# khangklj/Video2Music

Hardware: AMD Instinct MI355X
Metric: chord_tokens_per_sec_generated (higher is better)
Workload: dtype f32; 1 GPU; AMT 6+6 layers d_model=512 H=8 dff=1024 rpr, seq=1024, batch=32 clips/GPU x 300-frame video features (F=1287), feedback-greedy (G2) generate incl. video encode; global_batch=32, seq_len=1024, parallelism=dp1

## Files before the change

### include/amt_hip.h

```cpp
#ifndef AMT_HIP_H
#define AMT_HIP_H
#include <stdint.h>

#define AMT_ABI_VERSION 14

#ifdef __cplusplus
extern "C" {
#endif

typedef struct amt_handle amt_handle;

typedef struct amt_config {
    int32_t n_layers;
    int32_t num_heads;
    int32_t d_model;
    int32_t dim_feedforward;
    int32_t max_sequence_video;
    int32_t max_sequence_chord;
    int32_t total_vf_dim;
    int32_t max_batch;
} amt_config;

const char* amt_last_error(void);
int32_t amt_abi_version(void);
// ... 75 lines not shown
typedef struct amt_decode_gemm_args {
    const float* x;  int32_t ldx;
    const float* x2; int32_t ldx2;
    int32_t K1, K;
    const float* w_low;  const float* bias_low;  const float* resid; int32_t relu;
    const float* w_high; const float* bias_high;
    int32_t n_low, n_high;
    int32_t pro;
    const float* fold_g; const float* fold_c; const float* ln_w; const float* ln_b;
    float* y_low; float* y_high;
    float* scratch_low; float* scratch_high;
    int32_t B; float eps;
} amt_decode_gemm_args;
int32_t amt_decode_gemm_ex_fwd(const amt_decode_gemm_args* a, void* stream);
int32_t amt_decode_gemm_ex_lean(const amt_decode_gemm_args* a);
int32_t amt_gqa_fwd(const float* query, const float* key, const float* value,
                    const float* wq, const float* bq, const float* wk, const float* bk, const float* wv, const float* bv,
                    const float* ln_w, const float* ln_b, const float* wo, const float* bo,
                    float* out, float* scratch, int32_t L, int32_t S, int32_t B, int32_t E, int32_t query_heads,
                    int32_t kv_heads, int32_t is_causal, float ln_eps, void* stream);
int32_t amt_gqa_rope_fwd(const float* query, const float* key, const float* value,
                         const float* wq, const float* bq, const float* wk, const float* bk, const float* wv, const float* bv,
                         const float* ln_w, const float* ln_b, const float* wo, const float* bo,
                         float* out, float* scratch, int32_t L, int32_t S, int32_t B, int32_t E, int32_t query_heads,
                         int32_t kv_heads, int32_t is_causal, float ln_eps, const float* rope_cache, int32_t cache_rows,
                         int32_t cache_half, void* stream);
int64_t amt_moe_scratch_floats(int32_t n_tok, int32_t d, int32_t dff, int32_t n_exp);
int32_t amt_moe_fwd(const float* x, const float* gate_w, const float* gate_b,
                    const float* w1, const float* b1, const float* wg, const float* bg, const float* w2, const float* b2,
                    const float* sw1, const float* sb1, const float* swg, const float* sbg, const float* sw2, const float* sb2,
// ... 191 lines not shown
```

### video2music_amd/_lib.py

```python
import ctypes as C
import os

_HERE = os.path.dirname(os.path.abspath(__file__))
LIB_PATH = os.environ.get("AMT_LIB") or os.path.join(_HERE, "lib", "libamt_hip.so")


class AmtError(RuntimeError):
    pass


class AmtConfig(C.Structure):
    _fields_ = [("n_layers", C.c_int32), ("num_heads", C.c_int32), ("d_model", C.c_int32),
                ("dim_feedforward", C.c_int32), ("max_sequence_video", C.c_int32),
                ("max_sequence_chord", C.c_int32), ("total_vf_dim", C.c_int32), ("max_batch", C.c_int32)]


_P = C.c_void_p
_I = C.c_int32
_F = C.c_float


class DecodeGemmArgs(C.Structure):
    _fields_ = [("x", _P), ("ldx", _I), ("x2", _P), ("ldx2", _I), ("K1", _I), ("K", _I),
                ("w_low", _P), ("bias_low", _P), ("resid", _P), ("relu", _I), ("w_high", _P), ("bias_high", _P),
# ... 41 lines not shown
    "amt_diff_subln_fwd": [_P, _P, _P, _P, _I, _I, _F, _F, _F, _P],
    "amt_add_fwd": [_P, _P, _P, C.c_int64, _P],
    "amt_row_scale_add_fwd": [_P, _P, _P, _P, _I, _I, _P],
    "amt_rope_fwd": [_P, _P, _P, _I, _I, _I, _I, _I, _P],
    "amt_rpr_attn_fwd": [_P, _P, _P, _P, _P, _I, _I, _I, _I, _I, _P],
    "amt_rpr_attn_nomask_fwd": [_P, _P, _P, _P, _P, _I, _I, _I, _I, _I, _P],
    "amt_cross_attn_fwd": [_P, _P, _P, _P, _I, _I, _I, _I, _I, _I, _P],
    "amt_attn_fwd": [_P, _P, _P, _P, C.POINTER(C.c_int64), _I, _I, _I, _I, _I, _I, _I, _F, _P],
    "amt_concat_features_fwd": [_P, _I, _P, _P, _I, _P, _I, _P, _I, _I, _P],
    "amt_chord_embed_fwd": [_P] * 9 + [_I, _I, _I, _P],
    "amt_attn_decode_fwd": [_P, _P, _P, _P, _P, _I, _I, _I, _I, _I, _I, _P],
    "amt_decode_linear_fwd": [_P, _P, _P, _P, _P, _P, _P, _P, _P, _I, _I, _I, _I, _F, _P],
    "amt_attn_decode_fold_fwd": [_P, _I] + [_P] * 10 + [_I, _I, _I, _I, _P, _I, _I, _I, _F, _F, _P],
    "amt_decode_gemm_ex_fwd": [C.POINTER(DecodeGemmArgs), _P],
    "amt_decode_gemm_ex_lean": [C.POINTER(DecodeGemmArgs)],
    "amt_gqa_fwd": [_P] * 15 + [_I] * 7 + [_F, _P],
    "amt_gqa_rope_fwd": [_P] * 15 + [_I] * 7 + [_F, _P, _I, _I, _P],
    "amt_moe_scratch_floats": [_I, _I, _I, _I],
    "amt_moe_fwd": [_P] * 19 + [_I] * 4 + [_P],
    "amt_moe_topk_scratch_floats": [_I, _I, _I, _I, _I],
    "amt_moe_topk_fwd": [_P] * 19 + [_I] * 5 + [_P],
    "amt_moe_train_scratch_floats": [_I, _I, _I, _I, _I, _I],
    "amt_moe_train_fwd": [_P] * 22 + [_I] * 6 + [_P],
    "amt_moe_bwd_ws_floats": [_I, _I, _I, _I, _I],
    "amt_moe_bwd": [_P] * 29 + [_I] * 8 + [_F, _P],
    "amt_moe_route_fwd": [_P, _P, _P, _P, _P, _I, _I, _I, _P],
    "amt_glu_expert_fwd": [_P] * 9 + [_I, _I, _I, _P],
    "amt_moe_combine_fwd": [_P, _P, _P, _P, _P, _F, _P, _I, _I, _P],
    "amt_moe_ep_dispatch_plan_fwd": [_P, _I, _I, _P, _P, _P, _P, _P],
    "amt_gather_rows_fwd": [_P, _P, _P, _I, _I, _P],
# ... 43 lines not shown
    "amt_diff_subln_bwd": [_P] * 10 + [_I, _I, _F, _F, _P],
    "amt_moe_train_fwd_balanced": [_P] * 22 + [_I] * 6 + [_P, _P, _F, _P],
    "amt_selective_scan_wide_ckpt_steps": [_I],
    "amt_selective_scan_wide_train_fwd": [_P, _I, _P, _I, _P, _P, _P, _P, _I, _P, _P, _I, _P, _I, _P, _I, _P, _I, _I, _I, _I, _I, _I, _P],
    "amt_selective_scan_wide_bwd_ws_floats": [_I, _I, _I, _I],
    "amt_selective_scan_wide_bwd": [_P, _I, _P, _I, _P, _I, _P, _P, _P, _P, _I, _P, _P, _I, _P, _I, _P, _P, _I, _P, _I, _P, _I, _P, _P, _I, _P, _P,
                                    _P, _I, _I, _I, _I, _I, _I, _P],
    "amt_silu_bwd": [_P, _P, _P, C.c_int64, _P],
}
_RESTYPES = {"amt_last_error": C.c_char_p, "amt_decode_step_bytes": C.c_int64, "amt_moe_scratch_floats": C.c_int64, "amt_moe_topk_scratch_floats": C.c_int64,
             "amt_v2_step_ws_floats": C.c_int64, "amt_v2_step_batch_ws_floats": C.c_int64, "amt_moe_ep_expert_scratch_floats": C.c_int64,
             "amt_chord_loss_ws_floats": C.c_int64, "amt_attn_bwd_ws_floats": C.c_int64, "amt_selective_scan_bwd_ws_floats": C.c_int64,
             "amt_dwconv1d_silu_bwd_ws_floats": C.c_int64, "amt_moe_train_scratch_floats": C.c_int64, "amt_moe_bwd_ws_floats": C.c_int64,
             "amt_glu_train_scratch_floats": C.c_int64, "amt_glu_bwd_ws_floats": C.c_int64,
             "amt_selective_scan_wide_bwd_ws_floats": C.c_int64}
_NO_STATUS = set(_RESTYPES) | {"amt_abi_version", "amt_v2_last_step_launches", "amt_gemm_route", "amt_attn_route", "amt_decode_gemm_ex_lean", "amt_moe_wgrad_splits",
                                  "amt_rmsnorm_bwd_blocks", "amt_diff_subln_bwd_blocks", "amt_selective_scan_wide_ckpt_steps"}

ABI_VERSION = 14

_lib = None


def load():
    global _lib
    if _lib is not None:
        return _lib
    import torch
    if not os.path.exists(LIB_PATH):
        raise AmtError(f"{LIB_PATH} is missing: the HIP extension is not built (run __graft_entry__.build()); "
                       "video2music_amd has no CPU fallback")
# ... 44 lines not shown
```

### video2music_amd/csrc/amt_api.hip

```cpp
#include <stdarg.h>
#include <stdio.h>
#include <stdlib.h>
#include <string.h>

#include <algorithm>
#include <map>
#include <string>
#include <vector>

#include "../../include/amt_hip.h"
#include "amt_common.h"
#include "kernels.h"

static thread_local char g_err[1024] = "";

void amt_set_error(const char* fmt, ...) {
    va_list ap;
    va_start(ap, fmt);
    vsnprintf(g_err, sizeof(g_err), fmt, ap);
    va_end(ap);
}

extern "C" const char* amt_last_error(void) { return g_err; }
extern "C" int32_t amt_abi_version(void) { return AMT_ABI_VERSION; }
// ... 54 lines not shown
    float* unif = nullptr;
    int use_unif = 0;
    int64_t *tokens = nullptr, *roots = nullptr, *attrs = nullptr;
    int genB = 0, genT = 0, genP = 0, beam = 0, mcN = 0, mcC = 2, steps_done = 0;
    int n_root = 15;
    bool chord_embed = false;
    bool causal_mask = true;
    const float* vis_resid = nullptr;
    int skip_mask = 0;
    bool fuse_head = true;
    bool short_attn = true;
    bool step_short = false;
    bool l0_tables = true;
    bool gemm_pipe = true;
    bool gemm_lean = true;
    bool scalar_stream = true;
    bool plain_chain = false;
    bool gen_active = false;
    struct GraphKey { int B, T, P, beam, mcN, mcC, S, nsteps, skip, pad, short_ctx, parity, gemm_pipe, spare, key_stream, gemm_front; float* logits; };
    struct GraphEntry { GraphKey key; hipGraphExec_t exec; hipGraph_t graph; };
    std::vector<GraphEntry> graphs;
    hipStream_t cap_stream = nullptr;
};

namespace {

template <typename T>
int32_t dev_alloc(amt_handle* h, T** out, size_t count) {
    void* p = nullptr;
    AMT_HIP(hipMalloc(&p, count * sizeof(T) + 256));
// ... 148 lines not shown
            a.fold_lnw = P.n3w; a.fold_lnb = P.n3b; a.xn = h->xa; a.new_kv = 1; a.k_new = Kc; a.v_new = Vc;
            a.eps = LN_EPS; a.q_scale = qscale;
        }
        if (l == 0 && fused_sp) {
            if ((rc = amt_launch_attn_decode_sample(a, *fused_sp, s))) return rc;
        } else if (!(h->skip_mask & 1)) {
            PROF_BEGIN();
            if ((rc = amt_launch_attn_decode(a, s))) return rc;
            PROF_END(0);
        }
        const float* r0 = l == 0 ? h->x_in : h->xa;
        DecodeGemmParams g1{};
        g1.B = B; g1.eps = LN_EPS; g1.scale = 1.f; g1.x = h->ob; g1.ldx = d; g1.x2 = r0; g1.ldx2 = d; g1.K1 = d; g1.K = 2 * d;
        g1.Wp = L.p_sao; g1.bias = L.sa_ob; g1.resid = r0; g1.ldr = d; g1.y = h->u1; g1.ldy = d;
        g1.n_split = d; g1.N = 2 * d; g1.Wp2 = L.pf_a; g1.bias2 = L.va + 2 * d; g1.y2 = h->qraw; g1.ldy2 = d;
        PROF_BEGIN();
        if ((rc = launch_step_gemm(h, g1, s))) return rc;
        PROF_END(2);
        AttnDecodeParams x{};
        x.k = Kx; x.v = Vx; x.o = h->ob; x.B = B; x.H = H; x.hd = hd; x.cap = h->kx_rows; x.n_keys = h->encS; x.lane_key_stream = h->scalar_stream ? 0 : 1;
        x.q = h->qraw; x.ldq = d; x.d = d; x.fold_u = h->u1; x.fold_g = L.va; x.fold_c = L.va + d;
        x.fold_lnw = L.n1w; x.fold_lnb = L.n1b; x.xn = h->xb; x.eps = LN_EPS; x.q_scale = qscale;
        if (!(h->skip_mask & 2)) {
            PROF_BEGIN();
            if ((rc = amt_launch_attn_decode(x, s))) return rc;
            PROF_END(1);
        }
        DecodeGemmParams g2{};
        g2.B = B; g2.eps = LN_EPS; g2.scale = 1.f; g2.x = h->ob; g2.ldx = d; g2.x2 = h->xb; g2.ldx2 = d; g2.K1 = d; g2.K = 2 * d;
        g2.Wp = L.p_cao; g2.bias = L.ca_ob; g2.resid = h->xb; g2.ldr = d; g2.y = h->u2; g2.ldy = d;
        g2.n_split = d; g2.N = d + dff; g2.Wp2 = L.pf_b; g2.bias2 = L.vb + 2 * dff; g2.y2 = h->hraw; g2.ldy2 = dff;
        PROF_BEGIN();
        if ((rc = launch_step_gemm(h, g2, s))) return rc;
        PROF_END(2);
        DecodeGemmParams g3{};
        g3.B = B; g3.eps = LN_EPS; g3.scale = 1.f; g3.pro = 1; g3.x = h->hraw; g3.ldx = dff; g3.x2 = h->u2; g3.ldx2 = d;
        g3.K1 = dff; g3.K = dff + d; g3.fold_g = L.vb; g3.fold_c = L.vb + dff; g3.ln_w = L.n2w; g3.ln_b = L.n2b;
// ... 79 lines not shown
                DecodeGemmParams c = f2;
                c.x = h->hb + k0; c.K = std::min(FFN_CHUNK, dff - k0); c.Wp = L.p_l2 + (size_t)cdiv(d, 16) * 16 * k0;
                if (k0) { c.bias = nullptr; c.resid = h->u3; }
                PROF_BEGIN();
                if ((rc = launch_step_gemm(h, c, s))) return rc;
                PROF_END(2);
            }
        }
    }
    return 0;
}

int32_t get_graph(amt_handle* h, int first_pos, int nsteps, float* logits_out, hipGraphExec_t* out) {
    const bool short_ctx = h->short_attn && first_pos + nsteps <= amt_attn_decode_stride(h->hd);
    amt_handle::GraphKey key{h->genB, h->genT, h->genP, h->beam, h->mcN, h->mcC, h->encS, nsteps, h->skip_mask | (h->fuse_head ? 4 : 0), h->use_unif,
                             short_ctx ? 1 : 0, first_pos & 1, h->gemm_pipe ? 1 : 0, h->l0_tables ? 1 : 0, h->scalar_stream ? 1 : 0, h->gemm_lean ? 1 : 0, logits_out};
    for (auto& g : h->graphs)
        if (memcmp(&g.key, &key, sizeof(key)) == 0) { *out = g.exec; return 0; }
    hipGraph_t graph;
    if (!h->cap_stream) AMT_HIP(hipStreamCreateWithFlags(&h->cap_stream, hipStreamNonBlocking));
    hipStream_t cs = h->cap_stream;
    AMT_HIP(hipStreamBeginCapture(cs, hipStreamCaptureModeThreadLocal));
    int32_t rc = 0;
    const bool fuse = h->fold && h->fuse_head && !(h->skip_mask & 1);
    h->step_short = short_ctx;
    for (int i = 0; i < nsteps && !rc; ++i) {
        const int step = first_pos + i;
        if (fuse && i > 0) {
            const SampleParams sp = sample_params(h, logits_out, nullptr, 0, step - 1);
            rc = enqueue_decoder_step_folded(h, cs, step, nullptr, &sp);
        } else {
// ... 156 lines not shown
        const size_t mb = (size_t)cdiv(h->maxB, 16) * 16;
        const size_t bd = mb * d;
        if ((rc = dev_alloc(h, &h->x_in, bd))) return rc;
        if ((rc = dev_alloc(h, &h->u1, bd))) return rc;
        if ((rc = dev_alloc(h, &h->u2, bd))) return rc;
        if ((rc = dev_alloc(h, &h->u3, bd))) return rc;
        if ((rc = dev_alloc(h, &h->xa, bd))) return rc;
        if ((rc = dev_alloc(h, &h->xb, bd))) return rc;
        if ((rc = dev_alloc(h, &h->xc, bd))) return rc;
        if ((rc = dev_alloc(h, &h->qb, bd))) return rc;
        if ((rc = dev_alloc(h, &h->ob, bd))) return rc;
        if ((rc = dev_alloc(h, &h->hb, mb * dff))) return rc;
        h->fold = !h->plain_chain && d % 32 == 0 && 2 * d <= 1536 && (dff + d) % 64 == 0 && dff + d <= 1536 && dff % 16 == 0;
        if (h->fold) {
            if ((rc = dev_alloc(h, &h->qraw, bd))) return rc;
            if ((rc = dev_alloc(h, &h->hraw, mb * dff))) return rc;
            if ((rc = dev_alloc(h, &h->qkvraw, 3 * bd))) return rc;
            const size_t nmax = (size_t)std::max(3 * d, dff), kmax = (size_t)std::max(d, dff);
            if ((rc = dev_alloc(h, &h->tWs, nmax * d))) return rc;
            if ((rc = dev_alloc(h, &h->tT, kmax * d))) return rc;
            if ((rc = dev_alloc(h, &h->tWc, nmax * kmax))) return rc;
            if ((rc = dev_alloc(h, &h->tComb, nmax * (kmax + d)))) return rc;
            if ((rc = dev_alloc(h, &h->tWs2, (size_t)VS * d))) return rc;
            if ((rc = dev_alloc(h, &h->vs, (size_t)6 * VS))) return rc;
            if ((rc = dev_alloc(h, &h->lraw, mb * VS))) return rc;
            if ((rc = dev_alloc(h, &h->tab_r, (size_t)h->n_root * 3 * d))) return rc;
            if ((rc = dev_alloc(h, &h->tab_a, (size_t)16 * 3 * d))) return rc;
            if ((rc = dev_alloc(h, &h->tab_k, (size_t)3 * d))) return rc;
            if ((rc = dev_alloc(h, &h->tab_cb, (size_t)3 * d))) return rc;
            if ((rc = dev_alloc(h, &h->tab_p, (size_t)h->Tcap * 3 * d))) return rc;
// ... 99 lines not shown
    }
    if (strcmp(name, "fuse_sampling_head") == 0) {
        h->fuse_head = value != 0;
        return 0;
    }
    if (strcmp(name, "short_context_attn") == 0) {
        h->short_attn = value != 0;
        return 0;
    }
    if (strcmp(name, "gemm_tile_pipeline") == 0) {
        h->gemm_pipe = value != 0;
        return 0;
    }
    if (strcmp(name, "gemm_scalar_front") == 0) {
        h->gemm_lean = value != 0;
        return 0;
    }
    if (strcmp(name, "layer0_kv_from_tables") == 0) {
        h->l0_tables = value != 0;
        return 0;
    }
    if (strcmp(name, "scalar_key_stream") == 0) {
        h->scalar_stream = value != 0;
        return 0;
    }
    if (strcmp(name, "profile_skip") == 0) {
        AMT_CHECK_ARG(value >= 0 && value < 4, "amt_set_option: profile_skip takes 0 (none), 1 (self-attention), 2 (cross-attention) or 3");
        h->skip_mask = value;
        return 0;
    }
// ... 285 lines not shown
```

### video2music_amd/csrc/attn_decode.hip

```cpp
#include <stdlib.h>

#include <atomic>

#include "amt_common.h"
#include "kernels.h"
#include "sample_device.h"

namespace {

constexpr int NW = 8;
constexpr int UNROLL = 4;

template <int HD>
struct Batch {
    float4 k[UNROLL], v[UNROLL], e[UNROLL];
};

__device__ __forceinline__ float4 ld4_stream(const float* p, bool nt) {
    typedef float v4 __attribute__((ext_vector_type(4)));
    if (nt) { v4 t = __builtin_nontemporal_load(reinterpret_cast<const v4*>(p)); return make_float4(t.x, t.y, t.z, t.w); }
    return ld4(p);
}

template <int HD, bool NT, int RS = HD>
// ... 317 lines not shown
                o4.x = ((pr.x + pa.x) + kv * wk.x + bb.x) + pp.x; o4.y = ((pr.y + pa.y) + kv * wk.y + bb.y) + pp.y;
                o4.z = ((pr.z + pa.z) + kv * wk.z + bb.z) + pp.z; o4.w = ((pr.w + pa.w) + kv * wk.w + bb.w) + pp.w;
                st4(q.x_next + (size_t)b * d + cc, o4);
            }
        }
    } else {
        const int d = p.d, col = h * HD + c * 4;
        const float* ub = p.fold_u + (size_t)b * d;
        float4 uv[UCH];
#pragma unroll
        for (int i = 0; i < UCH; ++i) {
            const int k = min((i * 64 + lane) * 4, d - 4);
            uv[i] = ld4(ub + k);
        }
        const float* raw = p.q + (size_t)b * p.ldq + col;
        const float4 rq = ld4(raw), gq = ld4(p.fold_g + col), cq = ld4(p.fold_c + col);
        float4 rk = kn4, gk = kn4, ck = kn4, rv = kn4, gv = kn4, cv = kn4;
        if (fresh) {
            rk = ld4(raw + d); gk = ld4(p.fold_g + d + col); ck = ld4(p.fold_c + d + col);
            rv = ld4(raw + 2 * d); gv = ld4(p.fold_g + 2 * d + col); cv = ld4(p.fold_c + 2 * d + col);
        }
        float4 rcs = make_float4(1.f, 0.f, 1.f, 0.f);
        if (FOLD == 3) rcs = ld4(p.rope + (size_t)(*p.rope_pos) * p.rope_dim + (col % p.rope_dim));
        if (FOLD == 4) rcs = ld4(p.rope + (size_t)t * p.rope_dim + (col % p.rope_dim));
        if (F1 || SHORT) load_kv<HD, NT>(b0, kb, vb, j0, sub, c4, SHORT ? n_keys : p.cap);
        if (RPR && fresh) load_er<HD>(b0, eb, j0, sub, c4, n_keys);
        if (own_er) e_own = ld4(p.Er + (size_t)(p.er_len - 1) * HD + c4);
        __builtin_amdgcn_sched_barrier(0);
        const float inv_d = 1.0f / (float)d;
        float s = 0.f;
#pragma unroll
        for (int i = 0; i < UCH; ++i)
            if ((i * 64 + lane) * 4 < d) s += (uv[i].x + uv[i].y) + (uv[i].z + uv[i].w);
        const float mean = wave_sum(s) * inv_d;
        float qq = 0.f;
#pragma unroll
        for (int i = 0; i < UCH; ++i) {
            if ((i * 64 + lane) * 4 < d) {
                const float dx = uv[i].x - mean, dy = uv[i].y - mean, dz = uv[i].z - mean, dw = uv[i].w - mean;
                qq += (dx * dx + dy * dy) + (dz * dz + dw * dw);
            }
        }
        const float rstd = rsqrtf(wave_sum(qq) * inv_d + p.eps);
// ... 277 lines not shown
    switch (p.hd) {
        case 16: launch_decode_sample<16>(p, sp, stream); break;
        case 32: launch_decode_sample<32>(p, sp, stream); break;
        case 64: launch_decode_sample<64>(p, sp, stream); break;
        case 128: launch_decode_sample<128>(p, sp, stream); break;
        default: AMT_CHECK_ARG(false, "attn_decode_sample: head_dim %d not in {16,32,64,128}", p.hd);
    }
    AMT_LAUNCH_CHECK();
    return 0;
}

int32_t amt_launch_attn_decode(const AttnDecodeParams& p, hipStream_t stream) {
    AMT_CHECK_ARG(p.B > 0 && p.H > 0 && p.cap > 0, "attn_decode: bad shape B=%d H=%d cap=%d", p.B, p.H, p.cap);
    AMT_CHECK_ARG(p.pos != nullptr || (p.n_keys > 0 && p.n_keys <= p.cap), "attn_decode: n_keys=%d outside (0,%d]", p.n_keys, p.cap);
    AMT_CHECK_ARG(p.Er == nullptr || p.er_len + 1 >= p.cap, "attn_decode: er_len=%d smaller than the key capacity %d", p.er_len, p.cap);
    if (p.fold_u) {
        AMT_CHECK_ARG(p.fold_g && p.fold_c && p.d == p.H * p.hd && p.d % 4 == 0 && p.d <= UCH_MAX * 256 && p.ldq >= p.d && p.ldq % 4 == 0,
                      "attn_decode: bad folded prologue (d=%d ldq=%d)", p.d, p.ldq);
        AMT_CHECK_ARG(!p.xn || (p.fold_lnw && p.fold_lnb), "attn_decode: xn needs the LayerNorm affine");
        AMT_CHECK_ARG(!p.new_kv || (p.pos && p.k_new && p.v_new && p.ldq >= 3 * p.d), "attn_decode: new_kv needs pos, the cache and 3d raw columns");
        if (p.new_kv && p.rope) {
            AMT_CHECK_ARG(!p.Er && p.rope_dim > 0 && p.rope_dim % 4 == 0, "attn_decode: the rotary self-attention takes no relative-position table");
            switch (p.hd) {
                case 16: launch_decode<16, 4>(p, stream); break;
                case 32: launch_decode<32, 4>(p, stream); break;
                case 64: launch_decode<64, 4>(p, stream); break;
                case 128: launch_decode<128, 4>(p, stream); break;
                default: AMT_CHECK_ARG(false, "attn_decode: head_dim %d not in {16,32,64,128}", p.hd);
            }
        } else if (p.new_kv) {
// ... 38 lines not shown
```

### video2music_amd/csrc/decode_gemm.hip

```cpp
#include <limits.h>
#include <stdlib.h>

#include <mutex>

#include "amt_common.h"
#include "kernels.h"

namespace {

constexpr int MAXB = 4096;
constexpr int XPAD = 8;

__global__ void pack_weight_kernel(const float* __restrict__ W, float* __restrict__ P, int N, int K, int ldw) {
    const int kt_n = K / 16;
    const size_t tile = blockIdx.x;
    const int nt = (int)(tile / kt_n), kt = (int)(tile % kt_n);
    const int lane = threadIdx.x;
    const int n = nt * 16 + (lane & 15), k = kt * 16 + 4 * (lane >> 4);
    float4 v = make_float4(0.f, 0.f, 0.f, 0.f);
    if (n < N) v = ld4(W + (size_t)n * ldw + k);
    st4(P + (tile * 64 + lane) * 4, v);
}

constexpr int NW = 16;
// ... 483 lines not shown
                const int hh = nn / p.hd, cc = nn - hh * p.hd;
                float* dst = (n < 2 * p.d) ? p.kcache : p.vcache;
                dst[(((size_t)row * p.H + hh) * p.cap + t) * p.hd + cc] = val;
            }
        }
    }
#ifdef AMT_STAMPS
    STAMP(6);
    if (p.stamps && tid == 0) {
        unsigned long long* o = p.stamps + ((size_t)blockIdx.y * gridDim.x + blockIdx.x) * 8;
        for (int i = 0; i < 8; ++i) o[i] = st_[i];
    }
#endif
}

int32_t device_ordinal(int* dev) {
    AMT_HIP(hipGetDevice(dev));
    AMT_CHECK_ARG(*dev >= 0 && *dev < 64, "decode_gemm: device ordinal %d out of range", *dev);
    return 0;
}

template <auto Kernel>
int32_t allow_big_lds() {
    static bool attr_set[64] = {false};
    static std::mutex mu;
    int dev = 0;
    if (int32_t rc = device_ordinal(&dev)) return rc;
    std::lock_guard<std::mutex> lock(mu);
    if (!attr_set[dev]) {
        AMT_HIP(hipFuncSetAttribute((const void*)Kernel, hipFuncAttributeMaxDynamicSharedMemorySize, 160 * 1024));
// ... 260 lines not shown
}

template <int KCH, bool FULL>
int32_t launch_variant(const DecodeGemmParams& p, size_t lds, hipStream_t stream) {
#ifdef AMT_EXPERIMENT
    if (p.pro == 1 && amt_tuning().exp_a == 1) return launch_one<KCH, FULL, Pro::Plain>(p, lds, stream);
#endif
    if (p.pro == 1) return launch_one<KCH, FULL, Pro::FoldedFfn>(p, lds, stream);
    if (p.pro == 2) { if constexpr (FULL && KCH >= 2) return launch_one<KCH, FULL, Pro::FoldedGlu>(p, lds, stream); }
    if (p.glu_gate) return launch_one<KCH, FULL, Pro::Glu>(p, lds, stream);
    if (p.ln_w && p.ln2_w) { if constexpr (KCH <= 4) return launch_one<KCH, FULL, Pro::LayerNorm2>(p, lds, stream); }
    if (p.ln_w) { if constexpr (KCH <= 4) return launch_one<KCH, FULL, Pro::LayerNorm>(p, lds, stream); }
    return launch_one<KCH, FULL, Pro::Plain>(p, lds, stream);
}

}

bool amt_decode_gemm_lean_ok(const DecodeGemmParams& p) {
    if (p.generic_front || p.serial_loop) return false;
    if (!p.x || !p.x2 || !p.Wp || p.B <= 0 || p.ldw != 0 || p.K1 <= 0 || p.K1 >= p.K || p.K1 % 256 != 0 || p.K % 256 != 0 || p.K > 1536 || p.K == 1280) return false;
    if (p.sel || p.n_groups > 1 || p.pos || p.mode != 0 || p.rope || p.glu_pair || p.glu_gate || p.ln2_w || p.xn) return false;
    if (p.pro == 1 ? !(p.fold_g && p.fold_c && p.ln_w && p.ln_b) : (p.pro != 0 || p.ln_w)) return false;
    if (p.n_split > 0 && p.n_split < p.N && !p.Wp2) return false;
    const unsigned long long lim = 1ull << 32, rows = (unsigned long long)(p.B - 1);
    const unsigned long long n_lo = p.n_split > 0 ? p.n_split : p.N, n_hi = p.N - n_lo;
    if ((rows * p.ldx + p.K1) * 4 >= lim || (rows * p.ldx2 + (p.K - p.K1)) * 4 >= lim) return false;
    if ((rows * p.ldy + n_lo) * 4 >= lim || (rows * p.ldy2 + n_hi) * 4 >= lim) return false;
    if ((n_lo + 15) / 16 * (p.n_split > 0 ? p.K1 : p.K) * 64 >= lim || (n_hi + 15) / 16 * p.K * 64 >= lim) return false;
    return true;
}
// ... 40 lines not shown
    AMT_CHECK_ARG(!p.glu_gate || p.pro == 2 || (!p.ln_w && p.pro == 0 && (!p.x2 || (p.K1 % 256 == 0 && p.K % 256 == 0 && p.n_groups <= 1 && !p.glu_only))),
                  "decode_gemm: the gated prologue takes no LayerNorm, and a second source only behind whole 256-column chunks");
    AMT_CHECK_ARG(!p.glu_pair || (p.N % 16 == 0 && p.mode == 0 && !p.resid && !p.rope && p.n_split == 0 && !p.sel && p.n_groups <= 1 && p.scale_cols == 0 &&
                                  !p.relu && p.ldy >= p.N / 2), "decode_gemm: the paired gate | up epilogue takes a plain product of N %% 16 == 0 columns");
    AMT_CHECK_ARG(!p.rope || (p.pos && p.rope_dim > 0 && p.rope_dim % 2 == 0 && p.rope_cols % 2 == 0 && p.n_split == 0), "decode_gemm: bad rotary epilogue");
    if (p.pro == 2) {
        AMT_CHECK_ARG(p.x2 && p.glu_gate && p.fold_g && p.fold_c && p.fold_g2 && p.fold_c2 && p.ln_w && p.ln_b && !p.resid && p.K1 % 256 == 0 &&
                      (p.K == 512 || p.K == 768 || p.K == 1024 || (p.K == 1536 && p.K - p.K1 >= 512)) && p.n_groups <= 1 && !p.sel && p.ldw == 0,
                      "decode_gemm: incomplete folded gated-FFN prologue (K1=%d K=%d)", p.K1, p.K);
    } else if (p.pro == 1) {
        AMT_CHECK_ARG(p.x2 && p.fold_g && p.fold_c && p.ln_w && p.ln_b && !p.resid, "decode_gemm: incomplete folded-FFN prologue");
    } else {
        AMT_CHECK_ARG(!p.ln_w || (!p.x2 && p.K <= 1024), "decode_gemm: the LayerNorm prologue takes a single source of K <= 1024");
    }
    AMT_CHECK_ARG(!p.ln2_w || (p.ln_w && p.ln_b && p.ln2_b && p.pro == 0 && !p.glu_gate), "decode_gemm: the second LayerNorm follows a first one");
    const int wide_grp = amt_tuning().wide_grouped;
    if (wide_grp > 0 && p.n_groups > 1 && !p.ln_w && p.pro == 0 && !p.rope && !p.x2 && p.mode == 0 && p.ldw == 0 && !p.sel &&
        (p.K == 512 || p.K == 1024) && cdiv(p.N, 16) * cdiv(p.B, MT) * p.n_groups > 256) {
        if (p.glu_gate) return p.K == 512 ? launch_wide<2, Pro::Glu, 2>(p, stream) : launch_wide<4, Pro::Glu, 2>(p, stream);
        return p.K == 512 ? launch_wide<2, Pro::Plain, 2>(p, stream) : launch_wide<4, Pro::Plain, 2>(p, stream);
    }
    const int wide_ntw = amt_tuning().wide_ntw;
    if (wide_ntw > 0 && p.N >= 4096 && !p.x2 && p.n_split == 0 && !p.sel && p.n_groups <= 1 && p.mode == 0 && !p.rope && !p.glu_gate && p.pro == 0 &&
        p.ldw == 0 && (p.K == 512 || p.K == 1024) && (!p.ln_w || p.ln_b) && !p.ln2_w) {
        const bool ln = p.ln_w != nullptr;
        if (p.K == 512 && p.B > MT && p.B <= 2 * MT && amt_tuning().wide_rb2) return ln ? launch_wide2<2, Pro::LayerNorm, 4>(p, stream) : launch_wide2<2, Pro::Plain, 4>(p, stream);
        if (p.K == 512) {
            if (wide_ntw == 7) return ln ? launch_wide<2, Pro::LayerNorm, 7>(p, stream) : launch_wide<2, Pro::Plain, 7>(p, stream);
            return ln ? launch_wide<2, Pro::LayerNorm, 4>(p, stream) : launch_wide<2, Pro::Plain, 4>(p, stream);
        }
// ... 25 lines not shown
```

### video2music_amd/csrc/kernels.h

```cpp
#pragma once
#include "amt_common.h"

struct GemmParams {
    const float* A; int lda;
    const float* W; int ldw;
    float* C; int ldc;
    int M, N, K;
    const float* bias;
    const float* resid; int ldr;
    const float* rowadd; int rowadd_period;
    float scale; int scale_cols;
    int relu;
    int sigmoid;
    int head_split, hs_seq, hs_seq_cap, hs_d, hs_hd, hs_heads;
    size_t hs_part_stride;
    const int* tile_group; size_t w_group_stride, bias_group_stride;
    const int* a_gather;
    const float* silu_mul; int ld_silu;
};
static inline GemmParams gemm_params(const float* A, int lda, const float* W, int ldw, float* C, int ldc,
                                     int M, int N, int K, const float* bias) {
    GemmParams p{};
    p.A = A; p.lda = lda; p.W = W; p.ldw = ldw; p.C = C; p.ldc = ldc; p.M = M; p.N = N; p.K = K; p.bias = bias;
    p.scale = 1.f; p.rowadd_period = 1;
// ... 50 lines not shown
    const float* q;
    const float* k; const float* v;
    float* o;
    int B, H, hd, cap;
    const int* pos;
    int n_keys;
    const float* Er; int er_len;
    const float* fold_u; const float* fold_g; const float* fold_c; const float* fold_lnw; const float* fold_lnb;
    float* xn; int ldq, d, new_kv; float eps, q_scale;
    float* k_new; float* v_new;
    unsigned long long* stamps;
    const float* rope; int rope_dim; const int* rope_pos;
    int short_ctx;
    int l0_tables;
    int lane_key_stream;
};
int32_t amt_launch_attn_decode(const AttnDecodeParams& p, hipStream_t stream);
void amt_attn_decode_scalar_stream(int on);
int amt_attn_decode_stride(int hd);
bool amt_attn_decode_tables_fit(int hd, int cap, int ra_rows);

int32_t amt_launch_pack_weight(const float* W, float* P, int N, int K, hipStream_t stream, int ldw = 0);
struct DecodeGemmFront {
    const float* x;
    const float* x2b;
    const float* Wp; const float* Wp2;
    const float* fold_g; const float* fold_c;
    const float* ln_wb; const float* ln_bb;
    unsigned x_row_bytes, x2_row_bytes;
    int B, K, K1, LD;
// ... 18 lines not shown
    const float* x2; int ldx2, K1;
    int pro; const float* fold_g; const float* fold_c;
    const float* fold_g2; const float* fold_c2;
    const float* Wp2; const float* bias2; float* y2; int ldy2, n_split;
    const int* sel; size_t sel_w_stride; int sel_b_stride;
    int ldw;
    int n_groups; size_t x_group_off, y_group_off;
    const float* glu_gate; int glu_only;
    int glu_pair;
    const float* rope; int rope_cols, rope_dim;
    const float* zero;
    const float* ln2_w; const float* ln2_b;
    unsigned long long* stamps;
    int serial_loop;
    int generic_front;
};
int32_t amt_launch_decode_gemm(const DecodeGemmParams& p, hipStream_t stream);
bool amt_decode_gemm_lean_ok(const DecodeGemmParams& p);
int32_t amt_decode_gemm_init();

int32_t amt_launch_moe_combine(const float* y_rows, const int32_t* slot_pos, const int32_t* idx, const float* wts, const float* shared,
                               float shared_scale, const float* resid, float* out, int n_tok, int d, hipStream_t stream, int dense_B = 0);
int32_t amt_launch_moe_route_plan(const float* x, const float* gate_w, const float* gate_b, int32_t* idx, float* wts, int32_t* plan_ints,
                                  int32_t* perm, int32_t* slot_pos, int32_t* tile_group, int n_tok, int d, int n_exp, int k, int Mp,
                                  hipStream_t stream, const float* sel_bias = nullptr, float update_rate = 0.f, float* bias_delta = nullptr);
int32_t amt_launch_moe_combine_k(const float* y_rows, const int32_t* slot_pos, const int32_t* idx, const float* wts, const float* shared,
                                 float* out, int n_tok, int d, int k, hipStream_t stream);
int32_t amt_launch_v2_decide_fused(const float* logits, int ld_logits, int32_t* state_dev, int64_t* tokens, int64_t* roots, int64_t* attrs,
                                   int B, int T, int n_primer, int beam, int max_conseq_N, int max_conseq_chord, float temperature,
                                   const float* uniforms, int chord_embed, const float* keys, const float* PR, const float* PA,
                                   const float* wkey, const float* bias, const float* pe, float* x_next, int d, hipStream_t stream);
int32_t amt_launch_moe_route_combine(const float* x, const float* gate_w, const float* gate_b, int n_exp, const float* y_all, const float* shared,
// ... 59 lines not shown
```

### video2music_amd/csrc/ops_api.hip

```cpp
#include <math.h>
#include <stdint.h>

#include "../../include/amt_hip.h"
#include "amt_common.h"
#include "kernels.h"

extern "C" int32_t amt_linear_fwd(const float* x, const float* w, const float* bias, const float* resid, float* y,
                                  int32_t M, int32_t N, int32_t K, int32_t relu, void* stream) {
    AMT_CHECK_ARG(x && w && y, "amt_linear_fwd: null pointer");
    GemmParams g = gemm_params(x, K, w, K, y, N, M, N, K, bias);
    g.resid = resid; g.ldr = N; g.relu = relu;
    return amt_launch_gemm(g, (hipStream_t)stream);
}

extern "C" int32_t amt_layernorm_fwd(const float* x, const float* resid, const float* w, const float* b, float* y,
                                     int32_t rows, int32_t dim, float eps, void* stream) {
    AMT_CHECK_ARG(x && y, "amt_layernorm_fwd: null pointer");
    return amt_launch_layernorm(x, resid, w, b, nullptr, nullptr, y, rows, dim, eps, (hipStream_t)stream);
}

extern "C" int32_t amt_rmsnorm_fwd(const float* x, const float* w, float* y, int32_t rows, int32_t dim, float eps, void* stream) {
    AMT_CHECK_ARG(x && y, "amt_rmsnorm_fwd: null pointer");
    return amt_launch_rmsnorm(x, w, y, rows, dim, eps, (hipStream_t)stream);
}
// ... 198 lines not shown
    int32_t rc;
    if ((rc = decode_gemm_ex_params(a, "amt_decode_gemm_ex_fwd", &g))) return rc;
    hipStream_t s = (hipStream_t)stream;
    const int Klow = a->x2 ? a->K1 : a->K;
    if ((rc = amt_launch_pack_weight(a->w_low, a->scratch_low, a->n_low, Klow, s))) return rc;
    if (a->n_high > 0 && (rc = amt_launch_pack_weight(a->w_high, a->scratch_high, a->n_high, a->K, s))) return rc;
    return amt_launch_decode_gemm(g, s);
}

extern "C" int32_t amt_decode_gemm_ex_lean(const amt_decode_gemm_args* a) {
    DecodeGemmParams g{};
    if (decode_gemm_ex_params(a, "amt_decode_gemm_ex_lean", &g)) return -1;
    return amt_decode_gemm_lean_ok(g) ? 1 : 0;
}

extern "C" int32_t amt_decode_linear_fwd(const float* x, const float* w, const float* bias, const float* ln_w, const float* ln_b,
                                         const float* resid, float* y, float* xn_out, float* w_packed_scratch,
                                         int32_t B, int32_t N, int32_t K, int32_t relu, float eps, void* stream) {
    AMT_CHECK_ARG(x && w && y && w_packed_scratch, "amt_decode_linear_fwd: null pointer");
    hipStream_t s = (hipStream_t)stream;
    if (!amt_tuning().prepacked) {
        int32_t rc = amt_launch_pack_weight(w, w_packed_scratch, N, K, s);
        if (rc) return rc;
    }
    DecodeGemmParams g{};
    g.x = x; g.ldx = K; g.Wp = w_packed_scratch; g.bias = bias; g.B = B; g.N = N; g.K = K;
    g.ln_w = ln_w; g.ln_b = ln_b; g.xn = xn_out; g.eps = eps; g.resid = resid; g.ldr = N; g.relu = relu;
    g.scale = 1.f; g.y = y; g.ldy = N;
    return amt_launch_decode_gemm(g, s);
}
// ... 1 lines not shown
```

Baseline: 135,300 chord-tokens/s.

## Split-K the decode G1 cross-query GEMM into partials summed inside attention

```diff
diff --git a/include/amt_hip.h b/include/amt_hip.h
--- a/include/amt_hip.h
+++ b/include/amt_hip.h
@@ -113,6 +113,13 @@
 } amt_decode_gemm_args;
 int32_t amt_decode_gemm_ex_fwd(const amt_decode_gemm_args* a, void* stream);
 int32_t amt_decode_gemm_ex_lean(const amt_decode_gemm_args* a);
+int32_t amt_decode_gemm_ex_split_fwd(const amt_decode_gemm_args* a, float* parts, void* stream);
+int32_t amt_decode_gemm_ex_split(const amt_decode_gemm_args* a);
+int32_t amt_attn_decode_fold_parts_fwd(const float* raw, int32_t ldq, const float* parts, int64_t part_stride, const float* q_bias,
+                                       const float* kcache, const float* vcache, const float* u, const float* fold_g,
+                                       const float* fold_c, const float* ln_w, const float* ln_b, float* xn_out, float* o,
+                                       int32_t B, int32_t H, int32_t hd, int32_t cap, int32_t n_keys, int32_t lane_stream,
+                                       float eps, float q_scale, void* stream);
 int32_t amt_gqa_fwd(const float* query, const float* key, const float* value,
                     const float* wq, const float* bq, const float* wk, const float* bk, const float* wv, const float* bv,
                     const float* ln_w, const float* ln_b, const float* wo, const float* bo,
diff --git a/video2music_amd/_lib.py b/video2music_amd/_lib.py
--- a/video2music_amd/_lib.py
+++ b/video2music_amd/_lib.py
@@ -79,6 +79,9 @@
     "amt_attn_decode_fold_fwd": [_P, _I] + [_P] * 10 + [_I, _I, _I, _I, _P, _I, _I, _I, _F, _F, _P],
     "amt_decode_gemm_ex_fwd": [C.POINTER(DecodeGemmArgs), _P],
     "amt_decode_gemm_ex_lean": [C.POINTER(DecodeGemmArgs)],
+    "amt_decode_gemm_ex_split_fwd": [C.POINTER(DecodeGemmArgs), _P, _P],
+    "amt_decode_gemm_ex_split": [C.POINTER(DecodeGemmArgs)],
+    "amt_attn_decode_fold_parts_fwd": [_P, _I, _P, C.c_int64] + [_P] * 10 + [_I] * 6 + [_F, _F, _P],
     "amt_gqa_fwd": [_P] * 15 + [_I] * 7 + [_F, _P],
     "amt_gqa_rope_fwd": [_P] * 15 + [_I] * 7 + [_F, _P, _I, _I, _P],
     "amt_moe_scratch_floats": [_I, _I, _I, _I],
@@ -152,7 +155,7 @@
              "amt_dwconv1d_silu_bwd_ws_floats": C.c_int64, "amt_moe_train_scratch_floats": C.c_int64, "amt_moe_bwd_ws_floats": C.c_int64,
              "amt_glu_train_scratch_floats": C.c_int64, "amt_glu_bwd_ws_floats": C.c_int64,
              "amt_selective_scan_wide_bwd_ws_floats": C.c_int64}
-_NO_STATUS = set(_RESTYPES) | {"amt_abi_version", "amt_v2_last_step_launches", "amt_gemm_route", "amt_attn_route", "amt_decode_gemm_ex_lean", "amt_moe_wgrad_splits",
+_NO_STATUS = set(_RESTYPES) | {"amt_abi_version", "amt_v2_last_step_launches", "amt_gemm_route", "amt_attn_route", "amt_decode_gemm_ex_lean", "amt_decode_gemm_ex_split", "amt_moe_wgrad_splits",
                                   "amt_rmsnorm_bwd_blocks", "amt_diff_subln_bwd_blocks", "amt_selective_scan_wide_ckpt_steps"}
 
 ABI_VERSION = 14
diff --git a/video2music_amd/csrc/amt_api.hip b/video2music_amd/csrc/amt_api.hip
--- a/video2music_amd/csrc/amt_api.hip
+++ b/video2music_amd/csrc/amt_api.hip
@@ -92,6 +92,8 @@
     bool l0_tables = true;
     bool gemm_pipe = true;
     bool gemm_lean = true;
+    bool g1_split = true;
+    float* g1_parts = nullptr;
     bool scalar_stream = true;
     bool plain_chain = false;
     bool gen_active = false;
@@ -270,6 +272,9 @@
         g1.B = B; g1.eps = LN_EPS; g1.scale = 1.f; g1.x = h->ob; g1.ldx = d; g1.x2 = r0; g1.ldx2 = d; g1.K1 = d; g1.K = 2 * d;
         g1.Wp = L.p_sao; g1.bias = L.sa_ob; g1.resid = r0; g1.ldr = d; g1.y = h->u1; g1.ldy = d;
         g1.n_split = d; g1.N = 2 * d; g1.Wp2 = L.pf_a; g1.bias2 = L.va + 2 * d; g1.y2 = h->qraw; g1.ldy2 = d;
+        g1.serial_loop = h->gemm_pipe ? 0 : 1; g1.generic_front = h->gemm_lean ? 0 : 1;
+        const bool split = h->g1_split && h->g1_parts && amt_decode_gemm_split_ok(g1);
+        if (split) g1.split_parts = h->g1_parts;
         PROF_BEGIN();
         if ((rc = launch_step_gemm(h, g1, s))) return rc;
         PROF_END(2);
@@ -277,6 +282,7 @@
         x.k = Kx; x.v = Vx; x.o = h->ob; x.B = B; x.H = H; x.hd = hd; x.cap = h->kx_rows; x.n_keys = h->encS; x.lane_key_stream = h->scalar_stream ? 0 : 1;
         x.q = h->qraw; x.ldq = d; x.d = d; x.fold_u = h->u1; x.fold_g = L.va; x.fold_c = L.va + d;
         x.fold_lnw = L.n1w; x.fold_lnb = L.n1b; x.xn = h->xb; x.eps = LN_EPS; x.q_scale = qscale;
+        if (split) { x.q_parts = h->g1_parts; x.q_part_stride = (size_t)B * d; x.q_bias = L.va + 2 * d; }
         if (!(h->skip_mask & 2)) {
             PROF_BEGIN();
             if ((rc = amt_launch_attn_decode(x, s))) return rc;
@@ -386,7 +392,7 @@
 int32_t get_graph(amt_handle* h, int first_pos, int nsteps, float* logits_out, hipGraphExec_t* out) {
     const bool short_ctx = h->short_attn && first_pos + nsteps <= amt_attn_decode_stride(h->hd);
     amt_handle::GraphKey key{h->genB, h->genT, h->genP, h->beam, h->mcN, h->mcC, h->encS, nsteps, h->skip_mask | (h->fuse_head ? 4 : 0), h->use_unif,
-                             short_ctx ? 1 : 0, first_pos & 1, h->gemm_pipe ? 1 : 0, h->l0_tables ? 1 : 0, h->scalar_stream ? 1 : 0, h->gemm_lean ? 1 : 0, logits_out};
+                             short_ctx ? 1 : 0, first_pos & 1, h->gemm_pipe ? 1 : 0, h->l0_tables ? 1 : 0, h->scalar_stream ? 1 : 0, (h->gemm_lean ? 1 : 0) | (h->g1_split ? 2 : 0), logits_out};
     for (auto& g : h->graphs)
         if (memcmp(&g.key, &key, sizeof(key)) == 0) { *out = g.exec; return 0; }
     hipGraph_t graph;
@@ -573,6 +579,7 @@
         h->fold = !h->plain_chain && d % 32 == 0 && 2 * d <= 1536 && (dff + d) % 64 == 0 && dff + d <= 1536 && dff % 16 == 0;
         if (h->fold) {
             if ((rc = dev_alloc(h, &h->qraw, bd))) return rc;
+            if ((rc = dev_alloc(h, &h->g1_parts, DECODE_GEMM_SPLIT_PARTS * bd))) return rc;
             if ((rc = dev_alloc(h, &h->hraw, mb * dff))) return rc;
             if ((rc = dev_alloc(h, &h->qkvraw, 3 * bd))) return rc;
             const size_t nmax = (size_t)std::max(3 * d, dff), kmax = (size_t)std::max(d, dff);
@@ -702,6 +709,10 @@
     }
     if (strcmp(name, "gemm_scalar_front") == 0) {
         h->gemm_lean = value != 0;
+        return 0;
+    }
+    if (strcmp(name, "g1_split_k") == 0) {
+        h->g1_split = value != 0;
         return 0;
     }
     if (strcmp(name, "layer0_kv_from_tables") == 0) {
diff --git a/video2music_amd/csrc/attn_decode.hip b/video2music_amd/csrc/attn_decode.hip
--- a/video2music_amd/csrc/attn_decode.hip
+++ b/video2music_amd/csrc/attn_decode.hip
@@ -355,7 +355,18 @@
             uv[i] = ld4(ub + k);
         }
         const float* raw = p.q + (size_t)b * p.ldq + col;
-        const float4 rq = ld4(raw), gq = ld4(p.fold_g + col), cq = ld4(p.fold_c + col);
+        float4 rq = ld4(raw);
+        const float4 gq = ld4(p.fold_g + col), cq = ld4(p.fold_c + col);
+        constexpr int QP = FOLD == 1 ? 8 : 1;
+        float4 qp[QP], qb4 = kn4;
+        if constexpr (FOLD == 1) {
+            if (p.q_parts) {
+                const float* pr = p.q_parts + (size_t)b * p.ldq + col;
+#pragma unroll
+                for (int i = 0; i < QP; ++i) qp[i] = ld4(pr + (size_t)i * p.q_part_stride);
+                qb4 = ld4(p.q_bias + col);
+            }
+        }
         float4 rk = kn4, gk = kn4, ck = kn4, rv = kn4, gv = kn4, cv = kn4;
         if (fresh) {
             rk = ld4(raw + d); gk = ld4(p.fold_g + d + col); ck = ld4(p.fold_c + d + col);
@@ -368,6 +379,13 @@
         if (RPR && fresh) load_er<HD>(b0, eb, j0, sub, c4, n_keys);
         if (own_er) e_own = ld4(p.Er + (size_t)(p.er_len - 1) * HD + c4);
         __builtin_amdgcn_sched_barrier(0);
+        if constexpr (FOLD == 1) {
+            if (p.q_parts) {
+#pragma unroll
+                for (int i = 0; i < QP; ++i) { rq.x += qp[i].x; rq.y += qp[i].y; rq.z += qp[i].z; rq.w += qp[i].w; }
+                rq.x += qb4.x; rq.y += qb4.y; rq.z += qb4.z; rq.w += qb4.w;
+            }
+        }
         const float inv_d = 1.0f / (float)d;
         float s = 0.f;
 #pragma unroll
@@ -675,6 +693,8 @@
     AMT_CHECK_ARG(p.B > 0 && p.H > 0 && p.cap > 0, "attn_decode: bad shape B=%d H=%d cap=%d", p.B, p.H, p.cap);
     AMT_CHECK_ARG(p.pos != nullptr || (p.n_keys > 0 && p.n_keys <= p.cap), "attn_decode: n_keys=%d outside (0,%d]", p.n_keys, p.cap);
     AMT_CHECK_ARG(p.Er == nullptr || p.er_len + 1 >= p.cap, "attn_decode: er_len=%d smaller than the key capacity %d", p.er_len, p.cap);
+    AMT_CHECK_ARG(!p.q_parts || (p.fold_u && !p.new_kv && !p.rope && p.q_bias && p.q_part_stride >= (size_t)(p.B - 1) * p.ldq + p.d),
+                  "attn_decode: the raw query in parts belongs to the plain folded prologue (bias and part stride given)");
     if (p.fold_u) {
         AMT_CHECK_ARG(p.fold_g && p.fold_c && p.d == p.H * p.hd && p.d % 4 == 0 && p.d <= UCH_MAX * 256 && p.ldq >= p.d && p.ldq % 4 == 0,
                       "attn_decode: bad folded prologue (d=%d ldq=%d)", p.d, p.ldq);
diff --git a/video2music_amd/csrc/decode_gemm.hip b/video2music_amd/csrc/decode_gemm.hip
--- a/video2music_amd/csrc/decode_gemm.hip
+++ b/video2music_amd/csrc/decode_gemm.hip
@@ -521,6 +521,124 @@
 #endif
 }
 
+constexpr int SW = 8;
+struct DecodeGemmSplitArgs {
+    const float* x; const float* x2; const float* Wp; const float* Wp2;
+    const float* bias; const float* resid; const float* zero;
+    float* y; float* y2; float* parts;
+    unsigned x_row_bytes, x2_row_bytes;
+    int B, mb, n_lo, n_hi;
+    int n_low, n_high, ldy, ldy2, ldr, relu, scale_cols;
+    float scale;
+    unsigned long long* stamps;
+};
+
+template <int KCH>
+__global__ __launch_bounds__(SW * 64) void decode_gemm_split_kernel(DecodeGemmSplitArgs f) {
+    static_assert(KCH == 2 || KCH == 4, "K is 512 or 1024");
+    constexpr int RC = KCH / 2, K1 = KCH * 128, LD = K1 + XPAD, KT1 = K1 / 16;
+    extern __shared__ __attribute__((aligned(16))) float smem[];
+#ifdef AMT_STAMPS
+    unsigned long long st_[8] = {0, 0, 0, 0, 0, 0, 0, 0};
+#endif
+    STAMP(0);
+    float* xs = smem;
+    float* red = smem + MT * LD;
+    const int tid = threadIdx.x, lane = tid & 63;
+    const int wv = __builtin_amdgcn_readfirstlane(tid >> 6);
+    const unsigned loff = (unsigned)lane * 16u;
+    const int id = (int)blockIdx.x;
+    const int unit = (id / (8 * f.mb)) * 8 + (id & 7);
+    if (unit >= f.n_lo + 2 * f.n_hi) return;
+    const int m0 = ((id >> 3) % f.mb) * MT;
+    const int fam = unit < f.n_lo ? 0 : unit < f.n_lo + f.n_hi ? 1 : 2;
+    const int nt = fam == 0 ? unit : fam == 1 ? unit - f.n_lo : unit - f.n_lo - f.n_hi;
+    const char* src = reinterpret_cast<const char*>(fam == 2 ? f.x2 : f.x);
+    const unsigned row_bytes = fam == 2 ? f.x2_row_bytes : f.x_row_bytes;
+    float4 v[2][RC], wt[KCH];
+#pragma unroll
+    for (int j = 0; j < 2; ++j) {
+        const char* xr = src + (unsigned)min(m0 + wv + 8 * j, f.B - 1) * row_bytes;
+#pragma unroll
+        for (int c = 0; c < RC; ++c) v[j][c] = ld4_s(xr + 1024 * c, loff);
+    }
+    asm volatile("" ::: "memory");
+    const int kt_n = fam == 0 ? KT1 : 2 * KT1;
+    const float* wb = (fam == 0 ? f.Wp : f.Wp2) + (size_t)nt * kt_n * 256;
+    const wbuf_t wr = __builtin_amdgcn_make_buffer_rsrc(const_cast<float*>(wb), 0, kt_n * 1024, 0x00020000);
+    const unsigned kt0 = (unsigned)((fam == 2 ? KT1 : 0) + wv * KCH);
+#pragma unroll
+    for (int i = 0; i < KCH; ++i) wt[i] = ld4_buf(wr, loff, (kt0 + i) * 1024u);
+    __builtin_amdgcn_sched_barrier(0);
+    STAMP(1);
+#pragma unroll
+    for (int j = 0; j < 2; ++j)
+#pragma unroll
+        for (int c = 0; c < RC; ++c) st4(xs + (wv + 8 * j) * LD + chunk_col(c, lane), v[j][c]);
+    STAMP(2);
+    __syncthreads();
+    STAMP(3);
+    const int el = tid & 63, er = (tid >> 6) & 3;
+    const int row = m0 + 4 * (el >> 4) + er, n = nt * 16 + (el & 15);
+    const bool live = tid < 256 && row < f.B && n < (fam == 0 ? f.n_low : f.n_high);
+    const bool has_b = live && fam == 0 && f.bias != nullptr, has_r = live && fam == 0 && f.resid != nullptr;
+    const float e_bias = *(has_b ? f.bias + n : f.zero);
+    const float e_res = *(has_r ? f.resid + (size_t)row * f.ldr + n : f.zero);
+    const float* xa = xs + (lane & 15) * LD + 4 * (lane >> 4) + wv * KCH * 16;
+    if (fam == 0) {
+        const f32x4 acc0 = tiles_pipelined<RC, Pro::Plain, 0>(xa, nullptr, 0, reinterpret_cast<const float4(&)[RC]>(wt[0]), 0.f, 0.f, 0, 0);
+        const f32x4 acc1 = tiles_pipelined<RC, Pro::Plain, 0>(xa + RC * 16, nullptr, 0, reinterpret_cast<const float4(&)[RC]>(wt[RC]), 0.f, 0.f, 0, 0);
+#ifdef AMT_STAMPS
+        if (acc0[0] + acc1[0] == 1.2345e-30f) st_[7] = 1;
+#endif
+        STAMP(4);
+        store_partials(red + (2 * wv) * 256, acc0, lane);
+        store_partials(red + (2 * wv + 1) * 256, acc1, lane);
+        __syncthreads();
+        STAMP(5);
+        if (live) {
+            float val = sum_partials(red, tid) + e_bias;
+            if (n < f.scale_cols) val *= f.scale;
+            val += e_res;
+            val = act(val, f.relu);
+            f.y[(size_t)row * f.ldy + n] = val;
+        }
+    } else {
+        const f32x4 acc = tiles_pipelined<KCH, Pro::Plain, 0>(xa, nullptr, 0, wt, 0.f, 0.f, 0, 0);
+#ifdef AMT_STAMPS
+        if (acc[0] == 1.2345e-30f) st_[7] = 1;
+#endif
+        STAMP(4);
+        if (fam == 1) {
+            store_partials(red + wv * 256, acc, lane);
+            __syncthreads();
+            STAMP(5);
+            if (live) {
+                float val = 0.f;
+#pragma unroll
+                for (int w = 0; w < SW; ++w) val += red[w * 256 + tid];
+                f.y2[(size_t)row * f.ldy2 + n] = val;
+            }
+        } else {
+            float* pw = f.parts + (size_t)wv * f.B * f.n_high;
+            const int pn = nt * 16 + (lane & 15);
+#pragma unroll
+            for (int rr = 0; rr < 4; ++rr) {
+                const int pr = m0 + 4 * (lane >> 4) + rr;
+                if (pr < f.B && pn < f.n_high) pw[(size_t)pr * f.n_high + pn] = acc[rr];
+            }
+            STAMP(5);
+        }
+    }
+#ifdef AMT_STAMPS
+    STAMP(6);
+    if (f.stamps && tid == 0) {
+        unsigned long long* o = f.stamps + (size_t)blockIdx.x * 8;
+        for (int i = 0; i < 8; ++i) o[i] = st_[i];
+    }
+#endif
+}
+
 int32_t device_ordinal(int* dev) {
     AMT_HIP(hipGetDevice(dev));
     AMT_CHECK_ARG(*dev >= 0 && *dev < 64, "decode_gemm: device ordinal %d out of range", *dev);
@@ -811,6 +929,29 @@
     return launch_one<KCH, FULL, Pro::Plain>(p, lds, stream);
 }
 
+template <int KCH>
+int32_t launch_split(const DecodeGemmParams& p, hipStream_t stream) {
+    DecodeGemmSplitArgs f{};
+    f.x = p.x; f.x2 = p.x2; f.Wp = p.Wp; f.Wp2 = p.Wp2; f.bias = p.bias; f.resid = p.resid; f.zero = p.zero;
+    f.y = p.y; f.y2 = p.y2; f.parts = p.split_parts;
+    f.x_row_bytes = (unsigned)p.ldx * 4u; f.x2_row_bytes = (unsigned)p.ldx2 * 4u;
+    f.B = p.B; f.mb = cdiv(p.B, MT); f.n_lo = p.n_split >> 4; f.n_hi = cdiv(p.N - p.n_split, 16);
+    f.n_low = p.n_split; f.n_high = p.N - p.n_split; f.ldy = p.ldy; f.ldy2 = p.ldy2; f.ldr = p.ldr; f.relu = p.relu;
+    f.scale_cols = p.scale_cols; f.scale = p.scale; f.stamps = p.stamps;
+    constexpr size_t lds = (size_t)(MT * (KCH * 128 + XPAD) + NW * 256) * sizeof(float);
+    static_assert(lds <= 64 * 1024, "the split form stays inside the default LDS limit");
+    const int units8 = cdiv(f.n_lo + 2 * f.n_hi, 8) * 8;
+    hipLaunchKernelGGL((decode_gemm_split_kernel<KCH>), dim3(units8 * f.mb), dim3(SW * 64), lds, stream, f);
+    AMT_LAUNCH_CHECK();
+    return 0;
+}
+
+}
+
+bool amt_decode_gemm_split_ok(const DecodeGemmParams& p) {
+    if (!amt_decode_gemm_lean_ok(p)) return false;
+    if (p.pro != 0 || p.n_split <= 0 || p.N - p.n_split <= 0 || !p.y2) return false;
+    return 2 * p.K1 == p.K && (p.K == 512 || p.K == 1024);
 }
 
 bool amt_decode_gemm_lean_ok(const DecodeGemmParams& p) {
@@ -881,6 +1022,7 @@
         AMT_CHECK_ARG(!p.ln_w || (!p.x2 && p.K <= 1024), "decode_gemm: the LayerNorm prologue takes a single source of K <= 1024");
     }
     AMT_CHECK_ARG(!p.ln2_w || (p.ln_w && p.ln_b && p.ln2_b && p.pro == 0 && !p.glu_gate), "decode_gemm: the second LayerNorm follows a first one");
+    if (p.split_parts && amt_decode_gemm_split_ok(p)) return p.K == 512 ? launch_split<2>(p, stream) : launch_split<4>(p, stream);
     const int wide_grp = amt_tuning().wide_grouped;
     if (wide_grp > 0 && p.n_groups > 1 && !p.ln_w && p.pro == 0 && !p.rope && !p.x2 && p.mode == 0 && p.ldw == 0 && !p.sel &&
         (p.K == 512 || p.K == 1024) && cdiv(p.N, 16) * cdiv(p.B, MT) * p.n_groups > 256) {
diff --git a/video2music_amd/csrc/kernels.h b/video2music_amd/csrc/kernels.h
--- a/video2music_amd/csrc/kernels.h
+++ b/video2music_amd/csrc/kernels.h
@@ -88,6 +88,7 @@
     int short_ctx;
     int l0_tables;
     int lane_key_stream;
+    const float* q_parts; size_t q_part_stride; const float* q_bias;
 };
 int32_t amt_launch_attn_decode(const AttnDecodeParams& p, hipStream_t stream);
 void amt_attn_decode_scalar_stream(int on);
@@ -136,8 +137,11 @@
     unsigned long long* stamps;
     int serial_loop;
     int generic_front;
+    float* split_parts;
 };
 int32_t amt_launch_decode_gemm(const DecodeGemmParams& p, hipStream_t stream);
+bool amt_decode_gemm_split_ok(const DecodeGemmParams& p);
+constexpr int DECODE_GEMM_SPLIT_PARTS = 8;
 bool amt_decode_gemm_lean_ok(const DecodeGemmParams& p);
 int32_t amt_decode_gemm_init();
 
diff --git a/video2music_amd/csrc/ops_api.hip b/video2music_amd/csrc/ops_api.hip
--- a/video2music_amd/csrc/ops_api.hip
+++ b/video2music_amd/csrc/ops_api.hip
@@ -236,6 +236,41 @@
     return amt_decode_gemm_lean_ok(g) ? 1 : 0;
 }
 
+extern "C" int32_t amt_decode_gemm_ex_split_fwd(const amt_decode_gemm_args* a, float* parts, void* stream) {
+    DecodeGemmParams g{};
+    int32_t rc;
+    if ((rc = decode_gemm_ex_params(a, "amt_decode_gemm_ex_split_fwd", &g))) return rc;
+    AMT_CHECK_ARG(parts, "amt_decode_gemm_ex_split_fwd: null parts buffer");
+    g.split_parts = parts;
+    hipStream_t s = (hipStream_t)stream;
+    const int Klow = a->x2 ? a->K1 : a->K;
+    if ((rc = amt_launch_pack_weight(a->w_low, a->scratch_low, a->n_low, Klow, s))) return rc;
+    if (a->n_high > 0 && (rc = amt_launch_pack_weight(a->w_high, a->scratch_high, a->n_high, a->K, s))) return rc;
+    return amt_launch_decode_gemm(g, s);
+}
+
+extern "C" int32_t amt_decode_gemm_ex_split(const amt_decode_gemm_args* a) {
+    DecodeGemmParams g{};
+    if (decode_gemm_ex_params(a, "amt_decode_gemm_ex_split", &g)) return -1;
+    return amt_decode_gemm_split_ok(g) ? 1 : 0;
+}
+
+extern "C" int32_t amt_attn_decode_fold_parts_fwd(const float* raw, int32_t ldq, const float* parts, int64_t part_stride, const float* q_bias,
+                                                  const float* kcache, const float* vcache, const float* u, const float* fold_g,
+                                                  const float* fold_c, const float* ln_w, const float* ln_b, float* xn_out, float* o,
+                                                  int32_t B, int32_t H, int32_t hd, int32_t cap, int32_t n_keys, int32_t lane_stream,
+                                                  float eps, float q_scale, void* stream) {
+    AMT_CHECK_ARG(raw && kcache && vcache && u && fold_g && fold_c && o, "amt_attn_decode_fold_parts_fwd: null pointer");
+    AMT_CHECK_ARG(!parts || (q_bias && part_stride > 0), "amt_attn_decode_fold_parts_fwd: parts need their stride and the bias");
+    AMT_CHECK_ARG(n_keys > 0 && n_keys <= cap, "amt_attn_decode_fold_parts_fwd: n_keys=%d outside (0,%d]", n_keys, cap);
+    AttnDecodeParams a{};
+    a.q = raw; a.ldq = ldq; a.k = kcache; a.v = vcache; a.o = o; a.B = B; a.H = H; a.hd = hd; a.cap = cap; a.d = H * hd;
+    a.n_keys = n_keys; a.lane_key_stream = lane_stream ? 1 : 0;
+    a.fold_u = u; a.fold_g = fold_g; a.fold_c = fold_c; a.fold_lnw = ln_w; a.fold_lnb = ln_b; a.xn = xn_out; a.eps = eps; a.q_scale = q_scale;
+    if (parts) { a.q_parts = parts; a.q_part_stride = (size_t)part_stride; a.q_bias = q_bias; }
+    return amt_launch_attn_decode(a, (hipStream_t)stream);
+}
+
 extern "C" int32_t amt_decode_linear_fwd(const float* x, const float* w, const float* bias, const float* ln_w, const float* ln_b,
                                          const float* resid, float* y, float* xn_out, float* w_packed_scratch,
                                          int32_t B, int32_t N, int32_t K, int32_t relu, float eps, void* stream) {
```

Result: no change. 136,600 chord-tokens/s, median of 6 (+1.0%).
